# RegulatoryGenomicsGroup/chicdiff

Hardware: AMD Instinct MI355X
Metric: interactions/sec NB-GLM Wald test (higher is better)
Workload: dtype f64; 1 GPU; synthetic 2000000 interactions x 8 samples (4v4), size factors + offsets(theta=0.5) + dispersions + Wald, design ~condition; rows_per_gpu=2000000, samples=8, global_rows=2000000, parallelism=rows-sharded x1, collectives=none (single rank), ranks_in_communicator=1

## Files before the change

chicdiff_amd/csrc/api.hip:

```cpp
#include <math.h>
#include <stdarg.h>
#include <stdio.h>
#include <stdlib.h>
#include <string.h>

#include <algorithm>
#include <mutex>
#include <thread>
#include <string>
#include <vector>
#include <unordered_set>

#include <dlfcn.h>

#include "common.h"
#include "prior_mc.h"

using namespace cd;

namespace cd {
struct ChinputCols {
    std::vector<int32_t> bait, oe, N;
    std::string error;
};
// ... 108 lines not shown
#define HIPCHK(c, call)                                                                              \
    do {                                                                                             \
        hipError_t e_ = (call);                                                                      \
        if (e_ != hipSuccess) return fail(c, CHICDIFF_E_HIP, "%s: %s", #call, hipGetErrorString(e_)); \
    } while (0)

extern "C" {

const char *chicdiff_hip_last_error(const chicdiff_hip_ctx *ctx) { return ctx ? ctx->err : g_create_err; }

void chicdiff_hip_default_opts(chicdiff_nbglm_opts *o) {
    o->minDisp = 1e-8;
    o->dispTol = 1e-6;
    o->kappa0 = 1.0;
    o->maxit = 100;
    o->betaMaxit = 100;
    o->betaTol = 1e-8;
    o->minmu = 0.5;
    o->outlierSD = 2.0;
    o->dispPriorVar = NAN;
    o->trendCoef[0] = o->trendCoef[1] = NAN;
    o->fitType = 0;
    o->_pad = 0;
}

int chicdiff_hip_set_option(chicdiff_hip_ctx *c, const char *name, int64_t value) {
    if (!c || !name) return CHICDIFF_E_INVALID;
    const std::string k(name);
    if (k == "line_search_spread" && value >= 0 && value <= 3) c->opt_spread = (int)value;
    else if (k == "line_search_min_waves" && (value == 0 || (value >= 2 && value <= 4))) c->opt_min_waves = (int)value;
    else if (k == "line_search_prio" && value >= 0 && value <= 100) c->opt_prio = (int)value;
    else if (k == "line_search_chunk" && (value == 0 || (value >= 8 && value <= 64))) c->opt_chunk = (int)value;
    else if (k == "line_search_classes_a" && value >= 0 && value <= 6) c->opt_classes_a = (int)value;
    else if (k == "line_search_schedule" && (value == 0 || value == 1)) c->opt_schedule = (int)value;
    else if (k == "line_search_deal" && value >= 0 && value <= 64) c->opt_deal = (int)value;
    else if (k == "local_trend_substitute" && (value == 0 || value == 1)) c->opt_no_local_substitute = value ? 0 : 1;
    else if (k == "sharded_trend_gather" && (value == 0 || value == 1)) c->opt_trend_gather = (int)value;
    else if (k == "theta_grid_concurrency" && value >= 1 && value <= 16) c->opt_grid_lanes = (int)value;
    else if (k == "host_copy_threads" && value >= 1 && value <= 64) c->opt_host_threads = (int)value;
    else if (k == "select_all_rounds" && (value == 0 || value == 1)) c->opt_select_rounds = (int)value;
    else if (k == "trend_one_launch_per_pass" && (value == 0 || value == 1)) c->opt_trend_multilaunch = (int)value;
    else if (k == "fault_inject" && value >= 0 && value <= 7) c->opt_fault = (int)value;
    else if (k == "trend_persistent_blocks" && value >= 0 && value <= 256) c->opt_trend_blocks = (int)value;
    else if (k == "fuse_offsets" && value >= 0 && value <= 2) c->opt_fuse_offsets = (int)value;
    else if (k == "bench_fake_world" && value >= 0 && value <= kGatherMaxWorld) {
        if (value > 1 && !getenv("CHICDIFF_BENCH_FAKE_WORLD"))
            return fail(c, CHICDIFF_E_INVALID, "set_option: bench_fake_world is a rehearsal hook of bench.py (CHICDIFF_BENCH_FAKE_WORLD unset)");
        c->opt_fake_world = (int)value;
    }
    else if (k == "trend_mad_in_kernel" && (value == 0 || value == 1)) c->opt_mad_in_kernel = (int)value;
    else return fail(c, CHICDIFF_E_INVALID, "set_option: unknown option or value (%s = %lld)", name, (long long)value);
    return CHICDIFF_OK;
}

int chicdiff_hip_create(chicdiff_hip_ctx **out, int32_t device) {
    if (!out) return fail(nullptr, CHICDIFF_E_INVALID, "ctx out pointer is NULL");
    *out = nullptr;
    int ndev = 0;
    hipError_t e = hipGetDeviceCount(&ndev);
    if (e != hipSuccess || ndev <= 0)
        return fail(nullptr, CHICDIFF_E_HIP, "no HIP device available (%s): the HIP path cannot run, and there is no CPU fallback",
                    e != hipSuccess ? hipGetErrorString(e) : "device count 0");
    if (device < 0 || device >= ndev) return fail(nullptr, CHICDIFF_E_INVALID, "device %d out of range [0,%d)", device, ndev);
    chicdiff_hip_ctx *c = new chicdiff_hip_ctx();
    c->device = device;
    if ((e = hipSetDevice(device)) != hipSuccess || (e = hipStreamCreateWithFlags(&c->own_stream, hipStreamNonBlocking)) != hipSuccess ||
        (e = hipHostMalloc((void **)&c->h_sc, sizeof(FitScalars))) != hipSuccess ||
// ... 1360 lines not shown
    for (int k = 0; k < lanes; k++)
        if (lane_rc[k]) return fail(c, lane_rc[k], "theta_grid: %s", c->lanes[k]->err[0] ? c->lanes[k]->err : "a concurrent fit failed");
    timing_collect(c);
    return CHICDIFF_OK;
}

}

extern "C" int chicdiff_hip_wald_pvalues_dev(chicdiff_hip_ctx *c, const double *d_stat, int64_t n, double *d_p) {
    if (!c) return CHICDIFF_E_INVALID;
    if (!d_stat || !d_p || n < 0) return fail(c, CHICDIFF_E_INVALID, "wald_pvalues: bad arguments");
    HIPCHK(c, hipSetDevice(c->device));
    if (n > 0) launch_pvalues(d_stat, n, d_p, c->stream);
    HIPCHK(c, hipStreamSynchronize(c->stream));
    return CHICDIFF_OK;
}

extern "C" int chicdiff_hip_selftest_math_dev(chicdiff_hip_ctx *c, int32_t op, const double *d_x, int64_t n, double *d_out) {
    if (!c) return CHICDIFF_E_INVALID;
    if (!d_x || !d_out || n < 0 || op < 0 || op > 8) return fail(c, CHICDIFF_E_INVALID, "selftest_math: bad arguments");
    HIPCHK(c, hipSetDevice(c->device));
    if (n > 0) launch_math_selftest(op, d_x, n, d_out, c->stream);
    HIPCHK(c, hipStreamSynchronize(c->stream));
    return CHICDIFF_OK;
}

extern "C" int chicdiff_hip_selftest_r_random(int32_t kind, uint32_t seed, double a, double b, int64_t n, double *out) {
    if (!out || n < 0 || kind < 0 || kind > 3) return CHICDIFF_E_INVALID;
    if (kind == 3 && !(a > 0 && b > 0)) return CHICDIFF_E_INVALID;
    RStream r(seed);
    for (int64_t i = 0; i < n; i++) out[i] = kind == 0 ? r.unif() : kind == 1 ? r.norm() : kind == 2 ? r.expo() : r.gamma(a, b);
    return CHICDIFF_OK;
}
extern "C" int chicdiff_hip_selftest_prior_mc(int32_t df, const double *hist40, double *dens_out, double *prior_var_out) {
    if (df < 1 || df > 3) return CHICDIFF_E_INVALID;
    const PmcTable &t = pmc_table(df);
    if (dens_out) memcpy(dens_out, t.dens, sizeof t.dens);
    if (prior_var_out) {
        if (!hist40) return CHICDIFF_E_INVALID;
        *prior_var_out = pmc_prior_var(hist40, t);
    }
    return CHICDIFF_OK;
}

extern "C" int chicdiff_hip_fragment_background_dev(chicdiff_hip_ctx *c, const int32_t *d_bait, const int32_t *d_oe, int64_t nru,
                                                    int32_t id_min, int32_t nid, const int64_t *d_midsum, int32_t S,
                                                    const double *d_sj, const double *d_si, const int32_t *d_tblb,
                                                    const int32_t *d_tlb, const double *d_T, int32_t ntblb, int32_t ntlb,
                                                    const double *distfun_host, double *d_bmean, double *d_tmean,
                                                    double *d_fullmean) {
    if (!c) return CHICDIFF_E_INVALID;
    if (!d_bait || !d_oe || !d_midsum || !d_sj || !d_si || !d_tblb || !d_tlb || !d_T || !distfun_host || nru < 0 || nid < 1 ||
        S < 1 || S > kMaxS || ntblb < 1 || ntlb < 1)
        return fail(c, CHICDIFF_E_INVALID, "fragment_background: bad arguments");
    HIPCHK(c, hipSetDevice(c->device));
    int rc = ensure_aux(c, sizeof(double) * 10 * kMaxS);
    if (rc) return rc;
    double *d_df = reinterpret_cast<double *>(c->aux);
    hipError_t e = hipMemcpyAsync(d_df, distfun_host, sizeof(double) * 10 * S, hipMemcpyHostToDevice, c->stream);
    timing_reset(c);
    if (e == hipSuccess && nru > 0) {
        Scope t(c, "fragment_background");
        launch_fragment_background(d_bait, d_oe, nru, id_min, nid, d_midsum, S, d_sj, d_si, d_tblb, d_tlb, d_T, ntblb, ntlb, d_df,
                                   d_bmean, d_tmean, d_fullmean, c->stream);
    }
    if (e == hipSuccess) e = hipStreamSynchronize(c->stream);
// ... 341 lines not shown
```

chicdiff_amd/csrc/common.h:

```cpp
#pragma once
#include <hip/hip_runtime.h>
#include <stdint.h>

#include "../../include/chicdiff_hip.h"
#include "fit_driver.h"
#include "fit_state.h"

namespace cd {

constexpr int kRedBlocks = 1024;

struct FitDims {
    int64_t n;
    int32_t S, p, nA, nB;
    uint64_t gmask;
};

struct FitWork {
    double *baseMean, *baseVar, *gm0, *gm1, *rough, *binit0, *binit1, *crow;
    double *dispGene, *dispFit, *dispMAP, *disp, *beta0, *beta1, *resid;
    int32_t *allZero, *geneIter, *mapIter, *outlier, *betaIter, *optimConv;
    int32_t *order;
    uint8_t *cls;
    int32_t *gridlist;
// ... 9 lines not shown
    const double *logfact;
};
constexpr int kLogFactN = 1024;
constexpr int kQueueBytes = 2048;
constexpr int kRowHdr = 32;
__host__ __device__ inline int64_t row_stride(int S) {
    const int64_t bytes = kRowHdr + (int64_t)S * 12;
    return bytes <= 64 ? 64 : (bytes + 127) / 128 * 128;
}
__device__ __forceinline__ double *row_hdr(char *rowpack, int64_t r, int S) { return reinterpret_cast<double *>(rowpack + r * row_stride(S)); }

struct Opts {
    double minDisp, dispTol, kappa0, betaTol, minmu, outlierSD, dispPriorVarIn, maxDisp, trendIn[2];
    int32_t maxit, betaMaxit;
    int32_t fit_type = 0;
    int32_t spread = 1;
    int32_t min_waves = 0;
    int32_t schedule = 1;
    int32_t deal = 0;
    int32_t chunk = 0;
    int32_t classes_a = 0;
    int32_t xim_here = 0;
    int32_t prio = 0;
    int32_t trend_blocks = 0;
};

constexpr int kSchedClasses = 6, kSchedBlocks = 1024;
inline void order_tiles(int64_t n, int64_t &nblk, int64_t &tile) {
    nblk = (n + 255) / 256;
    if (nblk > kSchedBlocks) nblk = kSchedBlocks;
    tile = ((n + nblk - 1) / nblk + 255) / 256 * 256;
    nblk = (n + tile - 1) / tile;
}
#ifdef __HIPCC__
__device__ __forceinline__ void order_hist_store(const unsigned int (&mine)[kSchedClasses], unsigned int *hist) {
    __shared__ unsigned int s_cnt[kSchedClasses];
    if (threadIdx.x < kSchedClasses) s_cnt[threadIdx.x] = 0;
    __syncthreads();
#pragma unroll
    for (int k = 0; k < kSchedClasses; k++) {
        unsigned int v = mine[k];
        for (int off = 32; off > 0; off >>= 1) v += __shfl_down(v, off);
        if ((threadIdx.x & 63) == 0 && v) atomicAdd(&s_cnt[k], v);
    }
    __syncthreads();
    if (threadIdx.x < kSchedClasses) hist[threadIdx.x * gridDim.x + blockIdx.x] = s_cnt[threadIdx.x];
}
#endif

struct FusedOffsets { const double *fm = nullptr; const double *sf = nullptr; double theta = 0; int mix = 0; };
void launch_prep(const int32_t *counts, double *nf, FitDims d, FitWork w, Opts o, hipStream_t st, FusedOffsets fo = FusedOffsets());
void launch_prep_finish(FitDims d, FitWork w, double *slot, hipStream_t st);
void launch_xim(FitDims d, FitWork w, const double *slots, int world, hipStream_t st);
void launch_disp_gene(const int32_t *counts, const double *nf, FitDims d, FitWork w, Opts o, hipStream_t st);
void launch_order_build(FitDims d, FitWork w, int classesA, bool have_hist, hipStream_t st);
void launch_disp_map(const int32_t *counts, const double *nf, FitDims d, FitWork w, Opts o, hipStream_t st);
void launch_trend_persistent(FitDims d, FitWork w, Opts o, hipStream_t st, bool with_mad);
int trend_persistent_blocks();
void launch_trend_init(FitDims d, FitWork w, Opts o, hipStream_t st);
int trend_blocks();
void launch_trend_pass(FitDims d, FitWork w, Opts o, hipStream_t st, bool fused_step);
void launch_trend_step(FitDims d, FitWork w, Opts o, hipStream_t st);
constexpr int kLfMaxV = 100;
struct LfVerts { int nv; int _pad; double x[kLfMaxV], f[kLfMaxV], d[kLfMaxV]; };
void launch_lf_hist(FitDims d, FitWork w, Opts o, int use_dist, double xv, uint64_t prefix, int shift, double *hist, hipStream_t st);
void launch_lf_sums(FitDims d, FitWork w, Opts o, double xv, double h, double *partials, double *out8, hipStream_t st);
void launch_lf_eval(FitDims d, FitWork w, const LfVerts &v, hipStream_t st);
void launch_trend_gather(FitDims d, FitWork w, Opts o, double *xg, double *yg, hipStream_t st);
constexpr int kGatherMaxWorld = 64;
struct GatherLayout { int32_t world, _pad; int64_t block, maxn; int64_t off[kGatherMaxWorld + 1]; };
void launch_trend_compact(const GatherLayout &gl, const double *recv, double *xg, double *yg, hipStream_t st);
void launch_poke(int32_t *p, int32_t v, hipStream_t st);
void launch_flag_to_double(const int32_t *flag, double *out, hipStream_t st);
void launch_dispfit_resid(FitDims d, FitWork w, Opts o, hipStream_t st);
void launch_prior_var(FitDims d, FitWork w, Opts o, hipStream_t st);
void launch_resid_hist(FitDims d, FitWork w, double *out40, hipStream_t st);
void launch_prior_mc(FitDims d, FitWork w, const double *hist40, const void *table, hipStream_t st);
void launch_wald_prep(const int32_t *counts, const double *nf, FitDims d, FitWork w, Opts o, hipStream_t st);
void launch_wald_irls(const int32_t *counts, const double *nf, FitDims d, FitWork w, Opts o, hipStream_t st);
void launch_wald_final(const int32_t *counts, const double *nf, FitDims d, FitWork w, Opts o,
                       const chicdiff_nbglm_out &out, hipStream_t st);
void launch_wald_intercept(const int32_t *counts, const double *nf, FitDims d, FitWork w, Opts o,
                           const chicdiff_nbglm_out &out, hipStream_t st);
void launch_dev_sum_finish(FitDims d, FitWork w, const int32_t *carry, const double *sf_dev, hipStream_t st);

struct SelArgs {
    int mode;
    int ncol;
// ... 61 lines not shown
```

chicdiff_amd/csrc/disp_kernels.hip:

```cpp
#include <stdio.h>
#include <stdlib.h>

#include <vector>

#include "common.h"
#include "devmath.h"

namespace cd {

struct DD { double hi, lo; };
__device__ __forceinline__ void dd_add(DD &a, double x) {
    const double s = a.hi + x, bb = s - a.hi;
    a.lo += (a.hi - (s - bb)) + (x - bb);
    a.hi = s;
}
__device__ __forceinline__ void dd_add(DD &a, const DD &b) {
    dd_add(a, b.hi);
    a.lo += b.lo;
    const double s = a.hi + a.lo;
    a.lo = a.lo - (s - a.hi);
    a.hi = s;
}

struct CountProfile { unsigned int w0 = 0, w1 = 0, w2 = 0; };
// ... 199 lines not shown

__global__ void xim_kernel(FitDims d, FitWork w, const double *slots, int world) {
    if (threadIdx.x || blockIdx.x) return;
    if (slots)
        for (int j = 0; j <= d.S; j++) {
            DD a{0.0, 0.0};
            for (int r = 0; r < world; r++) dd_add(a, DD{slots[((size_t)r * (d.S + 1) + j) * 2], slots[((size_t)r * (d.S + 1) + j) * 2 + 1]});
            const double s = a.hi + a.lo;
            if (j < d.S) w.sc->colsum[j] = s; else w.sc->nnz = s;
        }
    double x = 0;
    for (int j = 0; j < d.S; j++) x += 1.0 / (w.sc->colsum[j] / w.sc->nnz);
    w.sc->xim = x / d.S;
}

constexpr int kColsumBlocks = 512;
static int prep16_blocks(int) { return 1024; }
void launch_prep(const int32_t *counts, double *nf, FitDims d, FitWork w, Opts, hipStream_t st, FusedOffsets fo) {
    if (d.S <= 16) {
        const int T = row_stride(d.S) > 128 ? 128 : 256;
        if (fo.fm) prep16_kernel<true><<<prep16_blocks(d.S), T, (size_t)T * (row_stride(d.S) + 4), st>>>(counts, nf, d, w, fo);
        else prep16_kernel<false><<<prep16_blocks(d.S), T, (size_t)T * (row_stride(d.S) + 4), st>>>(counts, nf, d, w, fo);
    } else {
        prep_kernel<<<kRedBlocks, 256, 0, st>>>(counts, nf, d, w);
        colsum_kernel<<<dim3(kColsumBlocks, d.S + 1), 256, 0, st>>>(nf, d, w);
    }
}
void launch_prep_finish(FitDims d, FitWork w, double *slot, hipStream_t st) {
    colsum_finish_kernel<<<d.S + 1, 64, 0, st>>>(d, w, d.S <= 16 ? prep16_blocks(d.S) : kColsumBlocks, d.S <= 16, slot);
}
void launch_xim(FitDims d, FitWork w, const double *slots, int world, hipStream_t st) { xim_kernel<<<1, 64, 0, st>>>(d, w, slots, world); }

constexpr int kSchedClassesA = 2, kSchedDeal = 8;
__device__ __forceinline__ int sched_class(double a0, double gmin, double minDisp) {
    if (!(a0 > 1.5 * minDisp)) return 5;
    const double s = a0 * gmin;
    return s < 0.1 ? 0 : (s < 0.316 ? 1 : (s < 1.0 ? 2 : (s < 3.16 ? 3 : (s < 10.0 ? 4 : 5))));
}
__global__ __launch_bounds__(256) void order_hist_kernel(const uint8_t *__restrict__ cls, int64_t n, int64_t tile, unsigned int *hist) {
    const int64_t lo = (int64_t)blockIdx.x * tile, hi = lo + tile < n ? lo + tile : n;
    unsigned int mine[kSchedClasses] = {0, 0, 0, 0, 0, 0};
    for (int64_t i = lo + threadIdx.x; i < hi; i += 256) {
        const int c = cls[i];
#pragma unroll
        for (int k = 0; k < kSchedClasses; k++) mine[k] += (c == k);
    }
    order_hist_store(mine, hist);
}
__global__ __launch_bounds__(256) void order_scatter_kernel(const uint8_t *__restrict__ cls, int64_t n, int64_t tile,
                                                            const unsigned int *__restrict__ hist, int32_t *__restrict__ order,
                                                            FitScalars *sc, int classesA) {
    __shared__ unsigned long long s_base[kSchedClasses + 1];
    __shared__ unsigned int s_wcnt[4][kSchedClasses];
    const int nblk = gridDim.x, lane = threadIdx.x & 63, wave = threadIdx.x >> 6;
    {
        unsigned long long part[kSchedClasses + 2] = {0, 0, 0, 0, 0, 0, 0, 0};
        const int total = kSchedClasses * nblk, cutA = classesA * nblk;
        for (int e = threadIdx.x; e < total; e += 256) {
            const unsigned long long hv = hist[e];
#pragma unroll
            for (int c = 0; c < kSchedClasses; c++) part[c] += e < c * nblk + (int)blockIdx.x ? hv : 0ull;
            part[kSchedClasses] += e < cutA ? hv : 0ull;
            part[kSchedClasses + 1] += hv;
        }
        __shared__ unsigned long long s_part[4][kSchedClasses + 2];
#pragma unroll
        for (int c = 0; c < kSchedClasses + 2; c++) {
            unsigned long long v = part[c];
            for (int off = 32; off > 0; off >>= 1) v += __shfl_down(v, off);
            if (lane == 0) s_part[wave][c] = v;
        }
        __syncthreads();
        if (threadIdx.x < kSchedClasses + 2) {
            const unsigned long long tot = s_part[0][threadIdx.x] + s_part[1][threadIdx.x] + s_part[2][threadIdx.x] + s_part[3][threadIdx.x];
            if (threadIdx.x < kSchedClasses) s_base[threadIdx.x] = tot;
            else if (blockIdx.x == 0) {
                if (threadIdx.x == kSchedClasses) sc->ord_na = (int64_t)tot;
                else sc->ord_n = (int64_t)tot;
            }
        }
        __syncthreads();
    }
    const int64_t lo = (int64_t)blockIdx.x * tile, hi = lo + tile < n ? lo + tile : n;
    for (int64_t i0 = lo; i0 < hi; i0 += 256) {
        const int64_t i = i0 + threadIdx.x;
        const int c = i < hi ? cls[i] : 255;
        unsigned int rank = 0;
#pragma unroll
        for (int k = 0; k < kSchedClasses; k++) {
            const unsigned long long m = __ballot(c == k);
            if (c == k) rank = __popcll(m & ((1ull << lane) - 1ull));
            if (lane == 0) s_wcnt[wave][k] = __popcll(m);
        }
        __syncthreads();
        if (c < kSchedClasses) {
            unsigned int before = 0;
            for (int w2 = 0; w2 < wave; w2++) before += s_wcnt[w2][c];
            order[s_base[c] + before + rank] = (int32_t)i;
        }
        __syncthreads();
        if (threadIdx.x < kSchedClasses) s_base[threadIdx.x] += s_wcnt[0][threadIdx.x] + s_wcnt[1][threadIdx.x] + s_wcnt[2][threadIdx.x] + s_wcnt[3][threadIdx.x];
        __syncthreads();
    }
}

template <bool MAP>
__global__ __launch_bounds__(256) void disp_init_kernel(FitDims d, FitWork w, Opts o, int64_t tile, unsigned int *hist, int xim_here) {
    const FitScalars *sc = w.sc;
    const double c0 = sc->coefs[0], c1 = sc->coefs[1];
    double xim = 0.0;
    if (!MAP) {
        if (xim_here) {
            double x = 0;
            for (int j = 0; j < d.S; j++) x += 1.0 / (sc->colsum[j] / sc->nnz);
            xim = x / d.S;
            if (blockIdx.x == 0 && threadIdx.x == 0) w.sc->xim = xim;
        } else {
            xim = sc->xim;
        }
    }
    const double out_thr = MAP ? o.outlierSD * sqrt(sc->varLogDispEsts) : 0.0;
    unsigned int mine[kSchedClasses] = {0, 0, 0, 0, 0, 0};
    const int64_t lo = tile > 0 ? (int64_t)blockIdx.x * tile : (int64_t)blockIdx.x * 256;
    const int64_t hi = tile > 0 ? (lo + tile < d.n ? lo + tile : d.n) : d.n;
    const int64_t step = tile > 0 ? 256 : (int64_t)gridDim.x * 256;
    struct In { int az; double bm, a, b, g0, g1; };
    auto load_in = [&](int64_t i) {
        In r;
        r.az = w.allZero[i];
        r.bm = w.baseMean[i];
        if (!MAP) {
            r.a = w.baseVar[i];
            r.b = w.rough[i];
            r.g0 = w.gm0[i];
            r.g1 = w.gm1[i];
        } else {
            r.a = w.dispGene[i];
            r.b = sc->trend_local ? w.dispFit[i] : 0.0;
            r.g0 = r.g1 = 0.0;
        }
        return r;
    };
    int64_t i = lo + threadIdx.x;
    In nxt{};
    if (i < hi) nxt = load_in(i);
    for (; i < hi; i += step) {
        const In cur = nxt;
        if (i + step < hi) nxt = load_in(i + step);
        if (cur.az) {
            if (!MAP) {
                w.cls[i] = 255;
                w.dispGene[i] = NAN;
                w.geneIter[i] = 0;
            }
            continue;
        }
        const double bm = cur.bm;
        if (!MAP) {
            const double moments = (cur.a - xim * bm) / (bm * bm);
            const double a0 = fmin(fmax(o.minDisp, fmin(cur.b, moments)), o.maxDisp);
            const double g0 = cur.g0, g1 = cur.g1;
            reinterpret_cast<double2 *>(w.start)[2 * i] = make_double2(a0, log(a0));
            const int c = sched_class(a0, d.p == 2 ? fmin(g0, g1) : g0, o.minDisp);
            w.cls[i] = (uint8_t)c;
#pragma unroll
            for (int k = 0; k < kSchedClasses; k++) mine[k] += (c == k);
        } else {
            const double dg = cur.a, df = sc->trend_local ? cur.b : c0 + c1 / bm;
            const double ldf = log(df);
            w.dispFit[i] = df;
            const int is_out = log(dg) > ldf + out_thr;
            reinterpret_cast<double2 *>(w.start)[2 * i] = make_double2(dg > 0.1 * df ? log(dg) : ldf, ldf);
            reinterpret_cast<double2 *>(w.start)[2 * i + 1] = make_double2(dg, (double)is_out);
            w.outlier[i] = is_out;
            if (is_out) w.disp[i] = dg;
        }
    }
    if (!MAP && tile > 0) order_hist_store(mine, hist);
}

constexpr int kChunk = 64;
constexpr int kTabSlots = 10;
static inline size_t disp_lds_per_wave(int S) { return (size_t)kTabSlots * 64 * 8 + (size_t)S * 64 * 12 + 3 * 64 * 4; }
enum Phase : int { PH_NEED = 0, PH_INIT = 1, PH_SEARCH = 2, PH_DONE = 5 };

__device__ __forceinline__ double max_num(double x, double m) {
    double r;
    asm("v_max_f64 %0, %1, %2" : "=v"(r) : "v"(x), "v"(m));
    return r;
}
template <int Q>
__device__ __forceinline__ bool load_row_mu_fixed(const char *row, double *s_nf, int *s_y, int lane, uint64_t gmask, double minmu) {
    const double2 *p = reinterpret_cast<const double2 *>(row);
    const int4 *py = reinterpret_cast<const int4 *>(row + kRowHdr + 32 * Q);
    const double2 h0 = p[0];
    const int4 prof = *reinterpret_cast<const int4 *>(row + 16);
    double2 f[2 * Q];
    int4 y[Q];
#pragma unroll
    for (int k = 0; k < 2 * Q; k++) f[k] = p[2 + k];
#pragma unroll
    for (int k = 0; k < Q; k++) y[k] = py[k];
    uint32_t gbits = (uint32_t)gmask;
    asm volatile("" : "+s"(gbits));
#pragma unroll
    for (int k = 0; k < 2 * Q; k++) {
        s_nf[(2 * k) * 64 + lane] = max_num(f[k].x * (((gbits >> (2 * k)) & 1u) ? h0.y : h0.x), minmu);
        s_nf[(2 * k + 1) * 64 + lane] = max_num(f[k].y * (((gbits >> (2 * k + 1)) & 1u) ? h0.y : h0.x), minmu);
    }
#pragma unroll
    for (int k = 0; k < Q; k++) {
// ... 764 lines not shown
            DIAG(unsigned long long tm[5];)
            eval_point(s_nf, s_y, s_tab, lane, live ? k : 0, S, gmask, p2, a_eval, MAP, prior_mean, prior_isig, l_new, dl_new, alpha_new, s_logtab, s_exptab DIAG(, tm));
            __builtin_amdgcn_wave_barrier();
            s_tab[lane] = l_new;
            __builtin_amdgcn_fence(__ATOMIC_RELEASE, "wavefront");
            __builtin_amdgcn_wave_barrier();
            __builtin_amdgcn_fence(__ATOMIC_ACQUIRE, "wavefront");
            double gbest = -INFINITY;
            gbi = 0;
            for (int t = 0; t < 20; t++) {
                const double v = s_tab[20 * k + t];
                if (v > gbest) {
                    gbest = v;
                    gbi = t;
                }
            }
            __builtin_amdgcn_wave_barrier();
            if (stage == 0) ghat = (gbi == 19) ? ghi : glo + gbi * gstep;
        }
        if (live && pt == 0) {
            const double fa = (gbi == 19) ? ghat + gstep : (ghat - gstep) + gbi * (2.0 * gstep / 19.0);
            const double dd = fmin(fmax(exp(fa), o.minDisp), o.maxDisp);
            if (!MAP) {
                A.w.dispGene[r_k] = dd;
            } else {
                const double2 st1 = reinterpret_cast<const double2 *>(A.w.start)[2 * (int64_t)r_k + 1];
                A.w.dispMAP[r_k] = dd;
                A.w.disp[r_k] = st1.y != 0.0 ? st1.x : dd;
            }
        }
    }
}

void launch_order_build(FitDims d, FitWork w, int classesA, bool have_hist, hipStream_t st) {
    int64_t nblk, tile;
    order_tiles(d.n, nblk, tile);
    unsigned int *hist = reinterpret_cast<unsigned int *>(w.hist);
    if (!have_hist) order_hist_kernel<<<(unsigned)nblk, 256, 0, st>>>(w.cls, d.n, tile, hist);
    order_scatter_kernel<<<(unsigned)nblk, 256, 0, st>>>(w.cls, d.n, tile, hist, w.order, w.sc, classesA);
}

static void launch_disp(bool map, const int32_t *counts, const double *nf, FitDims d, FitWork w, Opts o,
                        hipStream_t st) {
    const bool sched = !map && o.schedule && (d.n > 65536 || o.schedule == 2);
    if (map) disp_init_kernel<true><<<kRedBlocks, 256, 0, st>>>(d, w, o, 0, nullptr, 0);
    else if (!sched) disp_init_kernel<false><<<kRedBlocks, 256, 0, st>>>(d, w, o, 0, nullptr, o.xim_here);
    else {
        int64_t nblk, tile;
        order_tiles(d.n, nblk, tile);
        disp_init_kernel<false><<<(unsigned)nblk, 256, 0, st>>>(d, w, o, tile, reinterpret_cast<unsigned int *>(w.hist), o.xim_here);
    }
    const size_t lds_per_wave = disp_lds_per_wave(d.S);
    int threads = 128;
    while (threads > 64 && lds_per_wave * (threads / 64) > 40 * 1024) threads >>= 1;
    const size_t lds = lds_per_wave * (threads / 64);
    int64_t waves_needed = (d.n + 63) / 64;
    int64_t blocks = (waves_needed + threads / 64 - 1) / (threads / 64);
    const int waves_per_block = threads / 64;
    int64_t blocks_per_cu = (int64_t)(160 * 1024 / (lds + 2048));
    const bool lds3 = (int64_t)(160 * 1024 / (lds + 2048)) * waves_per_block >= 12;
    const bool three = lds3 && (map ? d.n >= 750000 : (d.n >= 3000000 || (d.S <= 4 && d.n >= 1500000)));
    const int min_waves = (o.min_waves >= 2 && o.min_waves <= 4) ? o.min_waves : (three ? 3 : 2);
    const int64_t by_regs = (int64_t)(4 * min_waves) / waves_per_block;
    if (blocks_per_cu > by_regs) blocks_per_cu = by_regs;
    if (blocks_per_cu > 8) blocks_per_cu = 8;
    if (blocks_per_cu < 1) blocks_per_cu = 1;
    const int64_t max_blocks = 256 * blocks_per_cu;
    if (blocks > max_blocks) blocks = max_blocks;
    if (blocks < 1) blocks = 1;
    const double rows_per_lane = (double)d.n / (double)(blocks * threads);
    const bool deal_most = !map && o.schedule == 1 && o.classes_a == 0 && rows_per_lane >= 1.8 && rows_per_lane <= 8.0;
    const int classes_a = o.schedule == 2 ? 0 : (o.classes_a > 0 ? o.classes_a : (deal_most ? 5 : kSchedClassesA));
    if (sched) launch_order_build(d, w, classes_a, true, st);
    DispArgs A{counts, nf, d, w, o, nullptr, o.spread, sched ? w.order : nullptr, (deal_most && o.deal == 0) ? 4 : o.deal, 1, kChunk,
               w.gridlist, reinterpret_cast<unsigned int *>(w.queue + (map ? 24 : 16)), o.prio};
#ifdef CHICDIFF_DIAG
    const char *stamp_file = getenv("CHICDIFF_DISP_STAMPS");
    const size_t stamp_words = (size_t)blocks * (threads / 64) * kStampSlots;
    if (stamp_file) {
        (void)hipMalloc((void **)&A.stamps, stamp_words * 8);
        (void)hipMemsetAsync(A.stamps, 0, stamp_words * 8, st);
    }
#endif
    A.chunk = o.chunk > 0 ? o.chunk : (d.n <= 65536 ? 16 : kChunk);
    const int variant = min_waves;
#define LAUNCH(M, W) disp_fit_kernel<M, W><<<(unsigned)blocks, threads, lds, st>>>(A)
    if (map) {
        if (variant >= 4) LAUNCH(true, 4); else if (variant == 3) LAUNCH(true, 3); else LAUNCH(true, 2);
    } else {
        if (variant >= 4) LAUNCH(false, 4); else if (variant == 3) LAUNCH(false, 3); else LAUNCH(false, 2);
    }
#undef LAUNCH
    {
        int64_t gblocks = (d.n / 50 / 3 + 1 + 1) / 2;
        if (gblocks > 1536) gblocks = 1536;
        if (gblocks < 1) gblocks = 1;
        if (map) disp_grid_kernel<true><<<(unsigned)gblocks, 128, 2 * lds_per_wave, st>>>(A);
        else disp_grid_kernel<false><<<(unsigned)gblocks, 128, 2 * lds_per_wave, st>>>(A);
    }
#ifdef CHICDIFF_DIAG
    if (stamp_file) {
        (void)hipStreamSynchronize(st);
        std::vector<unsigned long long> h(stamp_words);
        (void)hipMemcpy(h.data(), A.stamps, h.size() * 8, hipMemcpyDeviceToHost);
        FILE *f = fopen(stamp_file, map ? "ab" : "wb");
        if (f) {
// ... 19 lines not shown
```

chicdiff_amd/hip.py:

```python
from __future__ import annotations

import ctypes as C
import os

import numpy as np

from .dist import ALLGATHER_FN, ALLREDUCE_FN

_HERE = os.path.dirname(os.path.abspath(__file__))
LIB_PATH = os.path.join(_HERE, "lib", "libchicdiff_hip.so")

ST_TREND_FAILED, ST_PRIORVAR_MC, ST_BETA_NONCONV, ST_ALLZERO_ROWS, ST_TREND_LOCAL = 1, 2, 4, 8, 16


EXPORTS = [
    "chicdiff_hip_create", "chicdiff_hip_destroy", "chicdiff_hip_last_error", "chicdiff_hip_set_stream",
    "chicdiff_hip_set_allreduce", "chicdiff_hip_set_allgather", "chicdiff_hip_last_refits", "chicdiff_hip_set_option", "chicdiff_hip_default_opts", "chicdiff_hip_size_factors_dev",
    "chicdiff_hip_offsets_dev", "chicdiff_hip_window_sums_dev", "chicdiff_hip_count_join_dev",
    "chicdiff_hip_fragment_background_dev", "chicdiff_hip_bh_adjust_dev", "chicdiff_hip_ihw_apply_dev",
    "chicdiff_hip_region_universe_count_dev", "chicdiff_hip_region_universe_fill_dev", "chicdiff_hip_region_universe_dev", "chicdiff_hip_count_table_dev",
    "chicdiff_hip_chinput_read", "chicdiff_hip_chinput_table_dev", "chicdiff_hip_region_avdist_dev",
    "chicdiff_hip_count_join_inner_dev", "chicdiff_hip_count_join_multi_dev",
    "chicdiff_hip_malloc", "chicdiff_hip_free", "chicdiff_hip_outstanding_allocations", "chicdiff_hip_memcpy_h2d", "chicdiff_hip_memcpy_d2h",
    "chicdiff_hip_rccl_unique_id", "chicdiff_hip_rccl_init", "chicdiff_hip_cooks_filter_dev",
    "chicdiff_hip_independent_filtering_dev",
    "chicdiff_hip_nbglm_fit_dev", "chicdiff_hip_nbglm_fit", "chicdiff_hip_wald_test_dev", "chicdiff_hip_theta_grid_dev",
    "chicdiff_hip_wald_pvalues_dev", "chicdiff_hip_selftest_math_dev", "chicdiff_hip_selftest_r_random",
    "chicdiff_hip_selftest_prior_mc", "chicdiff_hip_selftest_chinput", "chicdiff_hip_kernel_times", "chicdiff_hip_enable_timing",
]


class Opts(C.Structure):
    _fields_ = [("minDisp", C.c_double), ("dispTol", C.c_double), ("kappa0", C.c_double),
                ("maxit", C.c_int32), ("betaMaxit", C.c_int32), ("betaTol", C.c_double),
                ("minmu", C.c_double), ("outlierSD", C.c_double), ("dispPriorVar", C.c_double),
                ("trendCoef", C.c_double * 2), ("fitType", C.c_int32), ("_pad", C.c_int32)]


OUT_DOUBLE = ["baseMean", "baseVar", "dispGeneEst", "dispFit", "dispMAP", "dispersion", "log2FoldChange",
              "lfcSE", "stat", "pvalue", "intercept", "interceptSE", "deviance", "maxCooks"]
OUT_INT = ["dispGeneIter", "dispIter", "dispOutlier", "betaConv", "betaIter", "allZero", "cooksArgmax"]


class Out(C.Structure):
    _fields_ = [(k, C.c_void_p) for k in OUT_DOUBLE + OUT_INT]


class Scalars(C.Structure):
    _fields_ = [("trendCoef", C.c_double * 2), ("varLogDispEsts", C.c_double), ("dispPriorVar", C.c_double),
                ("sumDeviance", C.c_double), ("nAllZero", C.c_int64), ("trendOuterIter", C.c_int32),
                ("status", C.c_int32)]


class ResultsInfo(C.Structure):
    _fields_ = [("filterThreshold", C.c_double), ("filterTheta", C.c_double), ("alpha", C.c_double), ("index", C.c_int32),
                ("_pad", C.c_int32), ("theta", C.c_double * 50), ("numRej", C.c_double * 50), ("lowess", C.c_double * 50)]


class KernelTime(C.Structure):
    _fields_ = [("name", C.c_char_p), ("ms", C.c_double), ("launches", C.c_int32), ("_pad", C.c_int32), ("bytes", C.c_double)]
# ... 436 lines not shown
```

include/chicdiff_hip.h:

```cpp
#ifndef CHICDIFF_HIP_H
#define CHICDIFF_HIP_H

#include <stdint.h>

#ifdef __cplusplus
extern "C" {
#endif

#define CHICDIFF_OK 0
#define CHICDIFF_E_INVALID 1
#define CHICDIFF_E_HIP 2
#define CHICDIFF_E_NOMEM 3
#define CHICDIFF_E_COMM 4
#define CHICDIFF_E_NUMERIC 5

#define CHICDIFF_ST_TREND_FAILED 1
#define CHICDIFF_ST_PRIORVAR_MC 2
#define CHICDIFF_ST_BETA_NONCONV 4
#define CHICDIFF_ST_ALLZERO_ROWS 8
#define CHICDIFF_ST_TREND_LOCAL 16

typedef struct chicdiff_hip_ctx chicdiff_hip_ctx;

typedef int (*chicdiff_allreduce_fn)(void *user, void *dev_buf, int64_t count);
// ... 134 lines not shown
int chicdiff_hip_region_universe_fill_dev(chicdiff_hip_ctx *ctx, const int32_t *d_bait, const int32_t *d_oe, int64_t n,
                                          int32_t RUexpand, const int32_t *d_chr_of, int32_t maxfrag,
                                          const int64_t *d_region_ptr, int32_t *d_ru_bait, int32_t *d_ru_region,
                                          int32_t *d_ru_oe);
int chicdiff_hip_region_universe_dev(chicdiff_hip_ctx *ctx, const int32_t *d_baitID, const int32_t *d_oeID, int64_t n, int32_t RUexpand,
                                     const int32_t *d_chr_of, int32_t maxfrag, int64_t *d_region_ptr, int32_t *d_minOE,
                                     int32_t *d_maxOE, int32_t *d_ru_baitID, int32_t *d_ru_regionID, int32_t *d_ru_otherEndID,
                                     int64_t capacity, int64_t *total_host);

int chicdiff_hip_nbglm_fit_dev(chicdiff_hip_ctx *ctx, const int32_t *d_counts, const double *d_nf, int64_t n,
                               int32_t S, const int32_t *group, const chicdiff_nbglm_opts *opts,
                               const chicdiff_nbglm_out *d_out, chicdiff_nbglm_scalars *scalars);

int chicdiff_hip_nbglm_fit(chicdiff_hip_ctx *ctx, const int32_t *counts, const double *nf, int64_t n, int32_t S,
                           const int32_t *group, const chicdiff_nbglm_opts *opts, const chicdiff_nbglm_out *out,
                           chicdiff_nbglm_scalars *scalars);

int chicdiff_hip_wald_test_dev(chicdiff_hip_ctx *ctx, const int32_t *d_counts, const double *d_fullMean, int64_t n,
                               int32_t S, const int32_t *group, double theta, const chicdiff_nbglm_opts *opts,
                               const chicdiff_nbglm_out *d_out, chicdiff_nbglm_scalars *scalars, double *sf_host);

int chicdiff_hip_theta_grid_dev(chicdiff_hip_ctx *ctx, const int32_t *d_counts, const double *d_fullMean,
                                const double *sf_host, int64_t n, int32_t S, const double *thetas,
                                int32_t ntheta, const chicdiff_nbglm_opts *opts, double *deviances_host);

int chicdiff_hip_wald_pvalues_dev(chicdiff_hip_ctx *ctx, const double *d_stat, int64_t n, double *d_p);

int chicdiff_hip_selftest_math_dev(chicdiff_hip_ctx *ctx, int32_t op, const double *d_x, int64_t n, double *d_out);

int chicdiff_hip_selftest_chinput(const char *path, int32_t nthreads, int64_t cap, int32_t *bait, int32_t *oe, int32_t *N,
                                  int64_t *nrows, char *err, int32_t errcap);
int chicdiff_hip_selftest_r_random(int32_t kind, uint32_t seed, double a, double b, int64_t n, double *out);
int chicdiff_hip_selftest_prior_mc(int32_t df, const double *hist40, double *dens_out, double *prior_var_out);

typedef struct {
    const char *name;
    double ms;
    int32_t launches;
    int32_t _pad;
    double bytes;
} chicdiff_kernel_time;
int32_t chicdiff_hip_kernel_times(chicdiff_hip_ctx *ctx, chicdiff_kernel_time *out, int32_t cap);
int chicdiff_hip_enable_timing(chicdiff_hip_ctx *ctx, int32_t on);

#ifdef __cplusplus
}
#endif
#endif
```

Baseline: 549.8 million interactions/s.

## Refine dispersion scheduling classes to 23 bins and rebuild order scatter kernel

Replaces the six-class line-search scheduling bins with a 23-class scheme (log-spaced edges on alpha*mean, plus a min-dispersion slot) selectable by schedule mode. The order scatter kernel is rewritten so each wave handles a quarter of the tile, uses match-by-ballot peer ranking, and computes prefix bases from the per-block histogram with vectorised loads instead of per-iteration block barriers. The dispersion kernel now counts classes via shared atomics. Finer sorting is meant to group rows with similar iteration counts and cut wave divergence in the line search, at the cost of more histogram traffic and shared memory.

```diff
diff --git a/chicdiff_amd/csrc/api.hip b/chicdiff_amd/csrc/api.hip
--- a/chicdiff_amd/csrc/api.hip
+++ b/chicdiff_amd/csrc/api.hip
@@ -164,7 +164,7 @@
     else if (k == "line_search_prio" && value >= 0 && value <= 100) c->opt_prio = (int)value;
     else if (k == "line_search_chunk" && (value == 0 || (value >= 8 && value <= 64))) c->opt_chunk = (int)value;
     else if (k == "line_search_classes_a" && value >= 0 && value <= 6) c->opt_classes_a = (int)value;
-    else if (k == "line_search_schedule" && (value == 0 || value == 1)) c->opt_schedule = (int)value;
+    else if (k == "line_search_schedule" && value >= 0 && value <= 4 && value != 2) c->opt_schedule = (int)value;
     else if (k == "line_search_deal" && value >= 0 && value <= 64) c->opt_deal = (int)value;
     else if (k == "local_trend_substitute" && (value == 0 || value == 1)) c->opt_no_local_substitute = value ? 0 : 1;
     else if (k == "sharded_trend_gather" && (value == 0 || value == 1)) c->opt_trend_gather = (int)value;
@@ -1591,6 +1591,13 @@
     for (int64_t i = 0; i < n; i++) out[i] = kind == 0 ? r.unif() : kind == 1 ? r.norm() : kind == 2 ? r.expo() : r.gamma(a, b);
     return CHICDIFF_OK;
 }
+extern "C" int chicdiff_hip_selftest_sched_class(int32_t mode, double min_disp, const double *alpha_init, const double *group_mean, int64_t n,
+                                                 int32_t *cls_out, int32_t *bounds) {
+    if (n < 0 || (n > 0 && (!alpha_init || !group_mean || !cls_out)) || mode < 1 || mode > 4) return CHICDIFF_E_INVALID;
+    for (int64_t i = 0; i < n; i++) cls_out[i] = cd::sched_class(alpha_init[i], group_mean[i], min_disp, mode);
+    if (bounds) for (int a = 0; a <= 6; a++) bounds[a] = cd::sched_classes_a(a, mode);
+    return CHICDIFF_OK;
+}
 extern "C" int chicdiff_hip_selftest_prior_mc(int32_t df, const double *hist40, double *dens_out, double *prior_var_out) {
     if (df < 1 || df > 3) return CHICDIFF_E_INVALID;
     const PmcTable &t = pmc_table(df);
diff --git a/chicdiff_amd/csrc/common.h b/chicdiff_amd/csrc/common.h
--- a/chicdiff_amd/csrc/common.h
+++ b/chicdiff_amd/csrc/common.h
@@ -65,19 +65,56 @@
     tile = ((n + nblk - 1) / nblk + 255) / 256 * 256;
     nblk = (n + tile - 1) / tile;
 }
+constexpr int kSchedClassesFine = 23, kSchedEdgesFine = 21, kSchedMinDispSlot = 17;
+constexpr int kSchedSix = 3, kSchedMinDispLast = 4;
+__host__ __device__ inline int sched_class(double a0, double gmin, double minDisp, int mode) {
+    constexpr double edge[kSchedEdgesFine] = {0.0316, 0.0422, 0.0562, 0.0750, 0.1, 0.1334, 0.1778, 0.2371, 0.316, 0.4217, 0.5623,
+                                              0.7499, 1.0, 1.3335, 1.7783, 2.3714, 3.16, 4.2170, 5.6234, 7.4989, 10.0};
+    if (!(a0 > 1.5 * minDisp)) return (mode == kSchedSix || mode == kSchedMinDispLast) ? kSchedClassesFine - 1 : kSchedMinDispSlot;
+    const double s = a0 * gmin;
+    int f = 0;
+    if (mode == kSchedSix) {
+#pragma unroll
+        for (int k = 4; k < kSchedEdgesFine; k += 4) f += !(s < edge[k]) ? 4 : 0;
+        f += f > 0 ? 1 : 0;
+    } else {
+#pragma unroll
+        for (int k = 0; k < kSchedEdgesFine; k++) f += !(s < edge[k]) ? 1 : 0;
+    }
+    return f < kSchedMinDispSlot ? f : f + 1;
+}
+__host__ __device__ inline int sched_classes_a(int a, int mode) {
+    if (a <= 0) return 0;
+    if (a <= 3) return 1 + 4 * a;
+    if (a == 4) return kSchedMinDispSlot;
+    if (a == 5) return (mode == kSchedSix || mode == kSchedMinDispLast) ? kSchedClassesFine - 1 : kSchedMinDispSlot;
+    return kSchedClassesFine;
+}
 #ifdef __HIPCC__
-__device__ __forceinline__ void order_hist_store(const unsigned int (&mine)[kSchedClasses], unsigned int *hist) {
-    __shared__ unsigned int s_cnt[kSchedClasses];
-    if (threadIdx.x < kSchedClasses) s_cnt[threadIdx.x] = 0;
+template <int NC>
+__device__ __forceinline__ void order_hist_store(const unsigned int (&mine)[NC], unsigned int *hist) {
+    __shared__ unsigned int s_cnt[NC];
+    if (threadIdx.x < NC) s_cnt[threadIdx.x] = 0;
     __syncthreads();
 #pragma unroll
-    for (int k = 0; k < kSchedClasses; k++) {
+    for (int k = 0; k < NC; k++) {
         unsigned int v = mine[k];
         for (int off = 32; off > 0; off >>= 1) v += __shfl_down(v, off);
         if ((threadIdx.x & 63) == 0 && v) atomicAdd(&s_cnt[k], v);
     }
     __syncthreads();
-    if (threadIdx.x < kSchedClasses) hist[threadIdx.x * gridDim.x + blockIdx.x] = s_cnt[threadIdx.x];
+    if (threadIdx.x < NC) hist[threadIdx.x * kSchedBlocks + blockIdx.x] = s_cnt[threadIdx.x];
+}
+__device__ __forceinline__ void class_peers(int c, bool valid, int lane, unsigned int &rank, unsigned int &count) {
+    unsigned long long m = __ballot(valid);
+#pragma unroll
+    for (int b = 0; b < 5; b++) {
+        const bool bit = (c >> b) & 1;
+        const unsigned long long set = __ballot(bit);
+        m &= bit ? set : ~set;
+    }
+    rank = __popcll(m & ((1ull << lane) - 1ull));
+    count = __popcll(m);
 }
 #endif
 
@@ -86,7 +123,7 @@
 void launch_prep_finish(FitDims d, FitWork w, double *slot, hipStream_t st);
 void launch_xim(FitDims d, FitWork w, const double *slots, int world, hipStream_t st);
 void launch_disp_gene(const int32_t *counts, const double *nf, FitDims d, FitWork w, Opts o, hipStream_t st);
-void launch_order_build(FitDims d, FitWork w, int classesA, bool have_hist, hipStream_t st);
+void launch_order_build(FitDims d, FitWork w, int classesA, bool have_hist, hipStream_t st, bool fine = false);
 void launch_disp_map(const int32_t *counts, const double *nf, FitDims d, FitWork w, Opts o, hipStream_t st);
 void launch_trend_persistent(FitDims d, FitWork w, Opts o, hipStream_t st, bool with_mad);
 int trend_persistent_blocks();
diff --git a/chicdiff_amd/csrc/disp_kernels.hip b/chicdiff_amd/csrc/disp_kernels.hip
--- a/chicdiff_amd/csrc/disp_kernels.hip
+++ b/chicdiff_amd/csrc/disp_kernels.hip
@@ -255,75 +255,99 @@
 void launch_xim(FitDims d, FitWork w, const double *slots, int world, hipStream_t st) { xim_kernel<<<1, 64, 0, st>>>(d, w, slots, world); }
 
 constexpr int kSchedClassesA = 2, kSchedDeal = 8;
-__device__ __forceinline__ int sched_class(double a0, double gmin, double minDisp) {
-    if (!(a0 > 1.5 * minDisp)) return 5;
-    const double s = a0 * gmin;
-    return s < 0.1 ? 0 : (s < 0.316 ? 1 : (s < 1.0 ? 2 : (s < 3.16 ? 3 : (s < 10.0 ? 4 : 5))));
-}
+template <int NC>
 __global__ __launch_bounds__(256) void order_hist_kernel(const uint8_t *__restrict__ cls, int64_t n, int64_t tile, unsigned int *hist) {
     const int64_t lo = (int64_t)blockIdx.x * tile, hi = lo + tile < n ? lo + tile : n;
-    unsigned int mine[kSchedClasses] = {0, 0, 0, 0, 0, 0};
+    unsigned int mine[NC] = {};
     for (int64_t i = lo + threadIdx.x; i < hi; i += 256) {
         const int c = cls[i];
 #pragma unroll
-        for (int k = 0; k < kSchedClasses; k++) mine[k] += (c == k);
-    }
-    order_hist_store(mine, hist);
-}
+        for (int k = 0; k < NC; k++) mine[k] += (c == k);
+    }
+    order_hist_store<NC>(mine, hist);
+}
+template <int NC>
 __global__ __launch_bounds__(256) void order_scatter_kernel(const uint8_t *__restrict__ cls, int64_t n, int64_t tile,
                                                             const unsigned int *__restrict__ hist, int32_t *__restrict__ order,
                                                             FitScalars *sc, int classesA) {
-    __shared__ unsigned long long s_base[kSchedClasses + 1];
-    __shared__ unsigned int s_wcnt[4][kSchedClasses];
-    const int nblk = gridDim.x, lane = threadIdx.x & 63, wave = threadIdx.x >> 6;
-    {
-        unsigned long long part[kSchedClasses + 2] = {0, 0, 0, 0, 0, 0, 0, 0};
-        const int total = kSchedClasses * nblk, cutA = classesA * nblk;
-        for (int e = threadIdx.x; e < total; e += 256) {
-            const unsigned long long hv = hist[e];
+    static_assert(NC <= 32 && kSchedBlocks == 4 * 256, "8 threads per class sum 256 partial counts; class_peers() tells 32 classes apart");
+    __shared__ unsigned int s_m[NC][256];
+    __shared__ unsigned int s_edge[NC];
+    __shared__ unsigned int s_part[NC][8][2];
+    __shared__ unsigned int s_tot[NC], s_pre[NC];
+    __shared__ unsigned int s_wh[4][NC];
+    __shared__ unsigned int s_wbase[4][NC];
+    const int nblk = gridDim.x, t = threadIdx.x, lane = t & 63, wave = t >> 6, blk = blockIdx.x;
+    if (t < 4 * NC) (&s_wh[0][0])[t] = 0;
+    __syncthreads();
+    const int64_t lo = (int64_t)blk * tile, hi = lo + tile < n ? lo + tile : n;
+    const int64_t quarter = tile / 4;
+    const int64_t wlo = lo + wave * quarter, whi = wlo + quarter < hi ? wlo + quarter : hi;
+    for (int64_t i0 = wlo; i0 < whi; i0 += 64) {
+        const int64_t i = i0 + lane;
+        const int c = i < whi ? cls[i] : 255;
+        unsigned int rank, count;
+        class_peers(c, c < NC, lane, rank, count);
+        if (c < NC && rank == 0) atomicAdd(&s_wh[wave][c], count);
+    }
+    const int t_own = blk >> 2;
 #pragma unroll
-            for (int c = 0; c < kSchedClasses; c++) part[c] += e < c * nblk + (int)blockIdx.x ? hv : 0ull;
-            part[kSchedClasses] += e < cutA ? hv : 0ull;
-            part[kSchedClasses + 1] += hv;
-        }
-        __shared__ unsigned long long s_part[4][kSchedClasses + 2];
+    for (int c = 0; c < NC; c++) {
+        const uint4 v = *reinterpret_cast<const uint4 *>(hist + c * kSchedBlocks + 4 * t);
+        const unsigned int e0 = 4 * t < nblk ? v.x : 0u, e1 = 4 * t + 1 < nblk ? v.y : 0u, e2 = 4 * t + 2 < nblk ? v.z : 0u, e3 = 4 * t + 3 < nblk ? v.w : 0u;
+        s_m[c][t] = e0 + e1 + e2 + e3;
+        if (t == t_own) s_edge[c] = (4 * t < blk ? e0 : 0u) + (4 * t + 1 < blk ? e1 : 0u) + (4 * t + 2 < blk ? e2 : 0u);
+    }
+    __syncthreads();
+    if (t < NC * 8) {
+        const int c = t >> 3, j = t & 7;
+        unsigned int tot = 0, pre = 0;
 #pragma unroll
-        for (int c = 0; c < kSchedClasses + 2; c++) {
-            unsigned long long v = part[c];
-            for (int off = 32; off > 0; off >>= 1) v += __shfl_down(v, off);
-            if (lane == 0) s_part[wave][c] = v;
-        }
-        __syncthreads();
-        if (threadIdx.x < kSchedClasses + 2) {
-            const unsigned long long tot = s_part[0][threadIdx.x] + s_part[1][threadIdx.x] + s_part[2][threadIdx.x] + s_part[3][threadIdx.x];
-            if (threadIdx.x < kSchedClasses) s_base[threadIdx.x] = tot;
-            else if (blockIdx.x == 0) {
-                if (threadIdx.x == kSchedClasses) sc->ord_na = (int64_t)tot;
-                else sc->ord_n = (int64_t)tot;
-            }
-        }
-        __syncthreads();
-    }
-    const int64_t lo = (int64_t)blockIdx.x * tile, hi = lo + tile < n ? lo + tile : n;
-    for (int64_t i0 = lo; i0 < hi; i0 += 256) {
-        const int64_t i = i0 + threadIdx.x;
-        const int c = i < hi ? cls[i] : 255;
-        unsigned int rank = 0;
-#pragma unroll
-        for (int k = 0; k < kSchedClasses; k++) {
-            const unsigned long long m = __ballot(c == k);
-            if (c == k) rank = __popcll(m & ((1ull << lane) - 1ull));
-            if (lane == 0) s_wcnt[wave][k] = __popcll(m);
-        }
-        __syncthreads();
-        if (c < kSchedClasses) {
-            unsigned int before = 0;
-            for (int w2 = 0; w2 < wave; w2++) before += s_wcnt[w2][c];
-            order[s_base[c] + before + rank] = (int32_t)i;
-        }
-        __syncthreads();
-        if (threadIdx.x < kSchedClasses) s_base[threadIdx.x] += s_wcnt[0][threadIdx.x] + s_wcnt[1][threadIdx.x] + s_wcnt[2][threadIdx.x] + s_wcnt[3][threadIdx.x];
-        __syncthreads();
+        for (int k = 0; k < 8; k++) {
+            const int q = (k + j) & 7;
+            const uint4 v = reinterpret_cast<const uint4 *>(&s_m[c][32 * j])[q];
+            const int first = 32 * j + 4 * q;
+            tot += v.x + v.y + v.z + v.w;
+            pre += (first < t_own ? v.x : 0u) + (first + 1 < t_own ? v.y : 0u) + (first + 2 < t_own ? v.z : 0u) + (first + 3 < t_own ? v.w : 0u);
+        }
+        s_part[c][j][0] = tot;
+        s_part[c][j][1] = pre;
+    }
+    __syncthreads();
+    if (t < NC) {
+        unsigned int tot = 0, pre = s_edge[t];
+        for (int j = 0; j < 8; j++) {
+            tot += s_part[t][j][0];
+            pre += s_part[t][j][1];
+        }
+        s_tot[t] = tot;
+        s_pre[t] = pre;
+    }
+    __syncthreads();
+    if (t < 4 * NC) {
+        const int w = t / NC, c = t - w * NC;
+        unsigned int base = s_pre[c];
+        for (int k = 0; k < c; k++) base += s_tot[k];
+        for (int w2 = 0; w2 < w; w2++) base += s_wh[w2][c];
+        s_wbase[w][c] = base;
+    }
+    if (blk == 0 && t == 0) {
+        unsigned long long na = 0, all = 0;
+        for (int c = 0; c < NC; c++) {
+            na += c < classesA ? s_tot[c] : 0u;
+            all += s_tot[c];
+        }
+        sc->ord_na = (int64_t)na;
+        sc->ord_n = (int64_t)all;
+    }
+    __syncthreads();
+    for (int64_t i0 = wlo; i0 < whi; i0 += 64) {
+        const int64_t i = i0 + lane;
+        const int c = i < whi ? cls[i] : 255;
+        unsigned int rank, count;
+        class_peers(c, c < NC, lane, rank, count);
+        if (c < NC) order[s_wbase[wave][c] + rank] = (int32_t)i;
+        if (c < NC && rank == 0) atomicAdd(&s_wbase[wave][c], count);
     }
 }
 
@@ -343,7 +367,11 @@
         }
     }
     const double out_thr = MAP ? o.outlierSD * sqrt(sc->varLogDispEsts) : 0.0;
-    unsigned int mine[kSchedClasses] = {0, 0, 0, 0, 0, 0};
+    __shared__ unsigned int s_cnt[kSchedClassesFine];
+    if (!MAP && tile > 0) {
+        if (threadIdx.x < kSchedClassesFine) s_cnt[threadIdx.x] = 0;
+        __syncthreads();
+    }
     const int64_t lo = tile > 0 ? (int64_t)blockIdx.x * tile : (int64_t)blockIdx.x * 256;
     const int64_t hi = tile > 0 ? (lo + tile < d.n ? lo + tile : d.n) : d.n;
     const int64_t step = tile > 0 ? 256 : (int64_t)gridDim.x * 256;
@@ -384,10 +412,13 @@
             const double a0 = fmin(fmax(o.minDisp, fmin(cur.b, moments)), o.maxDisp);
             const double g0 = cur.g0, g1 = cur.g1;
             reinterpret_cast<double2 *>(w.start)[2 * i] = make_double2(a0, log(a0));
-            const int c = sched_class(a0, d.p == 2 ? fmin(g0, g1) : g0, o.minDisp);
+            const int c = sched_class(a0, d.p == 2 ? fmin(g0, g1) : g0, o.minDisp, o.schedule);
             w.cls[i] = (uint8_t)c;
-#pragma unroll
-            for (int k = 0; k < kSchedClasses; k++) mine[k] += (c == k);
+            if (tile > 0) {
+                unsigned int rank, count;
+                class_peers(c, true, threadIdx.x & 63, rank, count);
+                if (rank == 0) atomicAdd(&s_cnt[c], count);
+            }
         } else {
             const double dg = cur.a, df = sc->trend_local ? cur.b : c0 + c1 / bm;
             const double ldf = log(df);
@@ -399,7 +430,10 @@
             if (is_out) w.disp[i] = dg;
         }
     }
-    if (!MAP && tile > 0) order_hist_store(mine, hist);
+    if (!MAP && tile > 0) {
+        __syncthreads();
+        if (threadIdx.x < kSchedClassesFine) hist[threadIdx.x * kSchedBlocks + blockIdx.x] = s_cnt[threadIdx.x];
+    }
 }
 
 constexpr int kChunk = 64;
@@ -1230,12 +1264,17 @@
     }
 }
 
-void launch_order_build(FitDims d, FitWork w, int classesA, bool have_hist, hipStream_t st) {
+void launch_order_build(FitDims d, FitWork w, int classesA, bool have_hist, hipStream_t st, bool fine) {
     int64_t nblk, tile;
     order_tiles(d.n, nblk, tile);
     unsigned int *hist = reinterpret_cast<unsigned int *>(w.hist);
-    if (!have_hist) order_hist_kernel<<<(unsigned)nblk, 256, 0, st>>>(w.cls, d.n, tile, hist);
-    order_scatter_kernel<<<(unsigned)nblk, 256, 0, st>>>(w.cls, d.n, tile, hist, w.order, w.sc, classesA);
+    if (fine) {
+        if (!have_hist) order_hist_kernel<kSchedClassesFine><<<(unsigned)nblk, 256, 0, st>>>(w.cls, d.n, tile, hist);
+        order_scatter_kernel<kSchedClassesFine><<<(unsigned)nblk, 256, 0, st>>>(w.cls, d.n, tile, hist, w.order, w.sc, classesA);
+    } else {
+        if (!have_hist) order_hist_kernel<kSchedClasses><<<(unsigned)nblk, 256, 0, st>>>(w.cls, d.n, tile, hist);
+        order_scatter_kernel<kSchedClasses><<<(unsigned)nblk, 256, 0, st>>>(w.cls, d.n, tile, hist, w.order, w.sc, classesA);
+    }
 }
 
 static void launch_disp(bool map, const int32_t *counts, const double *nf, FitDims d, FitWork w, Opts o,
@@ -1267,9 +1306,9 @@
     if (blocks > max_blocks) blocks = max_blocks;
     if (blocks < 1) blocks = 1;
     const double rows_per_lane = (double)d.n / (double)(blocks * threads);
-    const bool deal_most = !map && o.schedule == 1 && o.classes_a == 0 && rows_per_lane >= 1.8 && rows_per_lane <= 8.0;
+    const bool deal_most = !map && o.schedule != 2 && o.classes_a == 0 && rows_per_lane >= 1.8 && rows_per_lane <= 8.0;
     const int classes_a = o.schedule == 2 ? 0 : (o.classes_a > 0 ? o.classes_a : (deal_most ? 5 : kSchedClassesA));
-    if (sched) launch_order_build(d, w, classes_a, true, st);
+    if (sched) launch_order_build(d, w, sched_classes_a(classes_a, o.schedule), true, st, true);
     DispArgs A{counts, nf, d, w, o, nullptr, o.spread, sched ? w.order : nullptr, (deal_most && o.deal == 0) ? 4 : o.deal, 1, kChunk,
                w.gridlist, reinterpret_cast<unsigned int *>(w.queue + (map ? 24 : 16)), o.prio};
 #ifdef CHICDIFF_DIAG
diff --git a/chicdiff_amd/hip.py b/chicdiff_amd/hip.py
--- a/chicdiff_amd/hip.py
+++ b/chicdiff_amd/hip.py
@@ -25,7 +25,7 @@
     "chicdiff_hip_rccl_unique_id", "chicdiff_hip_rccl_init", "chicdiff_hip_cooks_filter_dev",
     "chicdiff_hip_independent_filtering_dev",
     "chicdiff_hip_nbglm_fit_dev", "chicdiff_hip_nbglm_fit", "chicdiff_hip_wald_test_dev", "chicdiff_hip_theta_grid_dev",
-    "chicdiff_hip_wald_pvalues_dev", "chicdiff_hip_selftest_math_dev", "chicdiff_hip_selftest_r_random",
+    "chicdiff_hip_wald_pvalues_dev", "chicdiff_hip_selftest_math_dev", "chicdiff_hip_selftest_r_random", "chicdiff_hip_selftest_sched_class",
     "chicdiff_hip_selftest_prior_mc", "chicdiff_hip_selftest_chinput", "chicdiff_hip_kernel_times", "chicdiff_hip_enable_timing",
 ]
 
diff --git a/include/chicdiff_hip.h b/include/chicdiff_hip.h
--- a/include/chicdiff_hip.h
+++ b/include/chicdiff_hip.h
@@ -190,6 +190,8 @@
                                   int64_t *nrows, char *err, int32_t errcap);
 int chicdiff_hip_selftest_r_random(int32_t kind, uint32_t seed, double a, double b, int64_t n, double *out);
 int chicdiff_hip_selftest_prior_mc(int32_t df, const double *hist40, double *dens_out, double *prior_var_out);
+int chicdiff_hip_selftest_sched_class(int32_t mode, double min_disp, const double *alpha_init, const double *group_mean, int64_t n,
+                                      int32_t *cls_out, int32_t *bounds);
 
 typedef struct {
     const char *name;
```

New measurement: 559.4 million interactions/s (median of 6 runs). +1.7%, better.
